# selftok-team/SelftokTokenizer

Hardware: NVIDIA H100
Metric: images/sec encode+50-step decode, 256x256/512-tok (higher is better)
Workload: dtype fp16 (IEEE-half operands on wgmma, fp32 accumulate; encoder/VQ/tables fp32)

## Files before the change

### selftoktokenizer_b200/csrc/gemm_tc.cu

```cuda
#include "common.cuh"
#include "hopper.cuh"
#include "kernels.h"

#include <stdlib.h>

namespace stk {

namespace {

using namespace hop;

constexpr int BM = 128, BN = 256, BK = 64, WK = 16;
constexpr int A_TILE_BYTES = BM * BK * 2;
constexpr int B_TILE_BYTES = BN * BK * 2;
constexpr int CONSUMERS = 2;
constexpr int NUM_THREADS = CONSUMERS * 128 + 32;
constexpr int ACC = BN / 2;

template <int NSPLIT> struct Cfg {
  static constexpr int PLANES = NSPLIT == 3 ? 2 : 1;
  static constexpr int STAGE_BYTES = PLANES * (A_TILE_BYTES + B_TILE_BYTES);
  static constexpr int STAGES = NSPLIT == 3 ? 2 : 4;
  static constexpr int SMEM_BYTES = STAGES * STAGE_BYTES + 1024  + 256 ;
};

__device__ __forceinline__ void wgmma_tile(float (&d)[ACC], uint64_t da, uint64_t db, uint32_t acc, bool fp16) {
  if (fp16) wgmma_m64n256k16_ss_f16(d, da, db, acc);
  else wgmma_m64n256k16_ss_bf16(d, da, db, acc);
}

__device__ __forceinline__ float2 ldg2(const float* p) { return *reinterpret_cast<const float2*>(p); }

template <int MODE, bool GELU>
__device__ __forceinline__ void epilogue_tile(const Epilogue& e, const float (&acc)[ACC], int64_t row0, int64_t M, int col0, int N) {
  const bool per_row_gate = MODE == EPI_RESID && e.gate && (e.gate_period > 1 || e.tab_rows);
  const bool per_row_add = MODE == EPI_STORE && e.addtab;
  const bool fp16 = e.fp16 != 0;
  int orow[2], mrow[2];
  bool rvalid[2];
#pragma unroll
  for (int r = 0; r < 2; ++r) {
    const int64_t m = row0 + 8 * r;
    rvalid[r] = m < M;
    const int mi = (int)m;
    if (e.row_map && rvalid[r]) {
      orow[r] = e.row_map[mi];
    } else if (e.plan && rvalid[r]) {
      const int b = mi / e.rpb_in;
      const int n_img = e.rpb_out - (e.plan_ctx ? e.rpb_in : e.row_off);
      orow[r] = b * e.rpb_out + plan_slot_row(mi % e.rpb_in, e.plan[2 * b], e.plan[2 * b + 1], n_img, e.plan_ctx != 0);
    } else {
      orow[r] = e.rpb_in > 0 ? (mi / e.rpb_in) * e.rpb_out + e.row_off + (mi % e.rpb_in) : mi;
    }
    if (e.tab_rows && rvalid[r]) mrow[r] = e.tab_rows[mi];
    else mrow[r] = per_row_gate ? mi % e.gate_period : (per_row_add ? mi % e.add_period : 0);
  }
#pragma unroll
  for (int j = 0; j < BN / 8; ++j) {
    const int n = col0 + 8 * j;
    if (n >= N) continue;
    const float2 bias = e.bias ? ldg2(e.bias + n) : make_float2(0.f, 0.f);
    const float2 g0 = (MODE == EPI_RESID && e.gate && !per_row_gate) ? ldg2(e.gate + n) : make_float2(1.f, 1.f);
#pragma unroll
    for (int r = 0; r < 2; ++r) {
      if (!rvalid[r]) continue;
      float2 y = make_float2(acc[4 * j + 2 * r] + bias.x, acc[4 * j + 2 * r + 1] + bias.y);
      if (GELU) y = gelu_tanh_fast2(y);
      const int64_t o = (int64_t)orow[r] * e.ldo + n;
      if (MODE == EPI_RESID) {
        const float2 res = ldg2(e.resid + o);
        const float2 gt = per_row_gate ? ldg2(e.gate + (int64_t)mrow[r] * e.gate_ld + n) : g0;
        y.x = fmaf(gt.x, y.x, res.x); y.y = fmaf(gt.y, y.y, res.y);
      }
      if (MODE == EPI_SPLIT) {
        const uint32_t hi = pack2_sat16(y.x, y.y, fp16);
        *reinterpret_cast<uint32_t*>(e.out_hi + o) = hi;
        if (e.out_lo) {
          const float lx = y.x - __bfloat162float(__float2bfloat16_rn(y.x)), ly = y.y - __bfloat162float(__float2bfloat16_rn(y.y));
          *reinterpret_cast<uint32_t*>(e.out_lo + o) = pack2_sat16(lx, ly, false);
        }
      } else {
        if (per_row_add) {
          const float2 a = ldg2(e.addtab + (int64_t)mrow[r] * e.add_ld + n);
          y.x += a.x; y.y += a.y;
        }
        *reinterpret_cast<float2*>(e.out + o) = y;
      }
    }
  }
}

__device__ __forceinline__ void epilogue_dispatch(const Epilogue& e, const float (&acc)[ACC], int64_t row0, int64_t M, int col0, int N) {
  if (e.mode == EPI_RESID) epilogue_tile<EPI_RESID, false>(e, acc, row0, M, col0, N);
  else if (e.mode == EPI_SPLIT) {
    if (e.act == ACT_GELU) epilogue_tile<EPI_SPLIT, true>(e, acc, row0, M, col0, N);
    else epilogue_tile<EPI_SPLIT, false>(e, acc, row0, M, col0, N);
  } else {
    if (e.act == ACT_GELU) epilogue_tile<EPI_STORE, true>(e, acc, row0, M, col0, N);
    else epilogue_tile<EPI_STORE, false>(e, acc, row0, M, col0, N);
  }
}

struct TcMaps {
  CUtensorMap a_hi, a_lo, b_hi, b_lo;
};

struct GemmParams {
  int64_t M;
  int N, K;
  int fp16;
  Epilogue ep;
  int conv_C = 0, conv_H = 0, conv_W = 0, conv_stride = 1;
  int raster_gm = 4;
};

__device__ __forceinline__ void tile_coords(int t, int pm_tiles, int n_tiles, int GM, int& pm, int& n_blk) {
  const int per_group = GM * n_tiles;
  const int group = t / per_group;
  const int first = group * GM;
  const int gm = min(GM, pm_tiles - first);
  const int local = t - group * per_group;
  pm = first + local % gm;
  n_blk = local / gm;
}

template <int NSPLIT, int CL, bool FP16>
__global__ void __launch_bounds__(NUM_THREADS, 1)
gemm_tc_kernel(const __grid_constant__ TcMaps maps0, const __grid_constant__ TcMaps maps1, const GemmParams p0, const GemmParams p1) {
  static_assert(NSPLIT == 1 || !FP16, "the fp16 mode is single-pass");
  using C = Cfg<NSPLIT>;
  extern __shared__ uint8_t smem_raw[];
  const uint32_t smem_base = (smem_u32(smem_raw) + 1023u) & ~1023u;
  const uint32_t bar_base = smem_base + C::STAGES * C::STAGE_BYTES;
  auto full_bar = [&](int s) { return bar_base + 8u * s; };
  auto empty_bar = [&](int s) { return bar_base + 8u * (C::STAGES + s); };

  const int warp = threadIdx.x >> 5, lane = threadIdx.x & 31;
  const uint32_t rank = CL > 1 ? cluster_ctarank() : 0;
  const int pm_tiles0 = (int)((p0.M + CL * BM - 1) / (CL * BM)), n_tiles0 = (p0.N + BN - 1) / BN;
  const int pm_tiles1 = (int)((p1.M + CL * BM - 1) / (CL * BM)), n_tiles1 = (p1.N + BN - 1) / BN;
  const int tiles0 = pm_tiles0 * n_tiles0;
  const int num_tiles = tiles0 + pm_tiles1 * n_tiles1;
  const int cluster_id = blockIdx.x / CL, num_clusters = gridDim.x / CL;

  if (warp == CONSUMERS * 4 && lane == 0) {
    tma_prefetch_desc(&maps0.a_hi);
    tma_prefetch_desc(&maps0.b_hi);
    if (NSPLIT == 3) { tma_prefetch_desc(&maps0.a_lo); tma_prefetch_desc(&maps0.b_lo); }
    if (p1.M > 0) {
      tma_prefetch_desc(&maps1.a_hi);
      tma_prefetch_desc(&maps1.b_hi);
      if (NSPLIT == 3) { tma_prefetch_desc(&maps1.a_lo); tma_prefetch_desc(&maps1.b_lo); }
    }
    for (int s = 0; s < C::STAGES; ++s) { mbar_init(full_bar(s), 1); mbar_init(empty_bar(s), CONSUMERS * CL); }
    asm volatile("fence.mbarrier_init.release.cluster;" ::: "memory");
  }
  __syncthreads();
  if (CL > 1) cluster_sync_all();

  if (warp >= CONSUMERS * 4) {
    if (warp == CONSUMERS * 4 && lane == 0) {
      int stage = 0; uint32_t phase = 0;
      const uint64_t w_policy = l2_policy_evict_last();
      for (int t = cluster_id; t < num_tiles; t += num_clusters) {
        const bool second = t >= tiles0;
        const TcMaps& mp = second ? maps1 : maps0;
        const GemmParams& pp = second ? p1 : p0;
        int pm, n_blk;
        if (second) tile_coords(t - tiles0, pm_tiles1, n_tiles1, p1.raster_gm, pm, n_blk);
        else tile_coords(t, pm_tiles0, n_tiles0, p0.raster_gm, pm, n_blk);
        const int nk = (pp.K + BK - 1) / BK;
        const int m_row = (pm * CL + (int)rank) * BM;
        const int n_row = n_blk * BN + (int)rank * (BN / CL);
        const int chunks = pp.conv_C > 0 ? pp.conv_C / BK : 1;
        int cx = 0, cy = 0, cb = 0;
        if (pp.conv_C > 0) {
          cx = m_row % pp.conv_W;
          cy = (m_row / pp.conv_W) % pp.conv_H;
          cb = m_row / (pp.conv_W * pp.conv_H);
        }
        for (int kb = 0; kb < nk; ++kb) {
          mbar_wait(empty_bar(stage), phase ^ 1);
          const uint32_t sa = smem_base + stage * C::STAGE_BYTES;
          const uint32_t sb = sa + C::PLANES * A_TILE_BYTES + (uint32_t)rank * (B_TILE_BYTES / CL);
          const uint32_t fb = full_bar(stage);
          mbar_expect_tx(fb, C::STAGE_BYTES);
          if (pp.conv_C > 0) {
            const int tap = kb / chunks, c0 = (kb - tap * chunks) * BK;
            const int dy = tap / 3, dx = tap - dy * 3;
            int x0 = cx + dx - 1, y0 = cy + dy - 1, n0 = cb;
            if (pp.conv_stride == 2) { x0 = cx + (dx >> 1); y0 = cy + (dy >> 1); n0 = cb * 4 + (dy & 1) * 2 + (dx & 1); }
            tma_load_4d(sa, &mp.a_hi, fb, c0, x0, y0, n0);
            if (NSPLIT == 3) tma_load_4d(sa + A_TILE_BYTES, &mp.a_lo, fb, c0, x0, y0, n0);
          } else {
            tma_load_2d(sa, &mp.a_hi, fb, kb * BK, m_row);
            if (NSPLIT == 3) tma_load_2d(sa + A_TILE_BYTES, &mp.a_lo, fb, kb * BK, m_row);
          }
          if (CL > 1) {
            tma_load_2d_mc(sb, &mp.b_hi, fb, kb * BK, n_row, (uint16_t)((1u << CL) - 1), w_policy);
            if (NSPLIT == 3) tma_load_2d_mc(sb + B_TILE_BYTES, &mp.b_lo, fb, kb * BK, n_row, (uint16_t)((1u << CL) - 1), w_policy);
          } else {
            tma_load_2d_hint(sb, &mp.b_hi, fb, kb * BK, n_row, w_policy);
            if (NSPLIT == 3) tma_load_2d_hint(sb + B_TILE_BYTES, &mp.b_lo, fb, kb * BK, n_row, w_policy);
          }
          if (++stage == C::STAGES) { stage = 0; phase ^= 1; }
        }
      }
    }
  } else {
    const int wg = warp >> 2;
    const bool signaller = (threadIdx.x & 127) == 0;
    auto release = [&](int s) {
      if (!signaller) return;
      if (CL == 1) mbar_arrive(empty_bar(s));
      else for (int r = 0; r < CL; ++r) mbar_arrive_cluster(empty_bar(s), (uint32_t)r);
    };
    int stage = 0; uint32_t phase = 0;
    for (int t = cluster_id; t < num_tiles; t += num_clusters) {
      const bool second = t >= tiles0;
      int pm, n_blk;
      if (second) tile_coords(t - tiles0, pm_tiles1, n_tiles1, p1.raster_gm, pm, n_blk);
      else tile_coords(t, pm_tiles0, n_tiles0, p0.raster_gm, pm, n_blk);
      const int nk = ((second ? p1.K : p0.K) + BK - 1) / BK;
      float acc[ACC];
#pragma unroll
      for (int i = 0; i < ACC; ++i) acc[i] = 0.f;
      int prev = -1;
      for (int kb = 0; kb < nk; ++kb) {
        mbar_wait(full_bar(stage), phase);
        const uint32_t sa_hi = smem_base + stage * C::STAGE_BYTES + wg * (64 * 128);
        const uint32_t sa_lo = sa_hi + A_TILE_BYTES;
        const uint32_t sb_hi = smem_base + stage * C::STAGE_BYTES + C::PLANES * A_TILE_BYTES;
        const uint32_t sb_lo = sb_hi + B_TILE_BYTES;
        wgmma_fence();
#pragma unroll
        for (int k = 0; k < BK / WK; ++k) {
          const uint32_t koff = k * WK * 2;
          const uint64_t da_hi = make_smem_desc(sa_hi + koff), db_hi = make_smem_desc(sb_hi + koff);
          wgmma_tile(acc, da_hi, db_hi, (kb > 0 || k > 0) ? 1u : 0u, FP16);
          if (NSPLIT == 3) {
            const uint64_t da_lo = make_smem_desc(sa_lo + koff), db_lo = make_smem_desc(sb_lo + koff);
            wgmma_tile(acc, da_hi, db_lo, 1u, false);
            wgmma_tile(acc, da_lo, db_hi, 1u, false);
          }
        }
        wgmma_commit();
        wgmma_wait<1>();
        if (prev >= 0) release(prev);
        prev = stage;
        if (++stage == C::STAGES) { stage = 0; phase ^= 1; }
      }
      wgmma_wait<0>();
      fence_regs(acc);
      release(prev);
      const int wl = threadIdx.x & 127;
      const int64_t row0 = (int64_t)(pm * CL + (int)rank) * BM + wg * 64 + (wl >> 5) * 16 + ((wl & 31) >> 2);
      const int col0 = n_blk * BN + 2 * (wl & 3);
      if (!second) epilogue_dispatch(p0.ep, acc, row0, p0.M, col0, p0.N);
      else epilogue_dispatch(p1.ep, acc, row0, p1.M, col0, p1.N);
    }
  }
  if (CL > 1) cluster_sync_all();
}

typedef CUresult (*EncodeTiledFn)(CUtensorMap*, CUtensorMapDataType, cuuint32_t, void*, const cuuint64_t*, const cuuint64_t*,
                                  const cuuint32_t*, const cuuint32_t*, CUtensorMapInterleave, CUtensorMapSwizzle,
                                  CUtensorMapL2promotion, CUtensorMapFloatOOBfill);
EncodeTiledFn g_encode = nullptr;
constexpr int kMaxDev = 64;
int g_num_sms_dev[kMaxDev];
bool g_attr_dev[kMaxDev];
int g_raster_gm = 4;
int g_gemm_ctas = 2;

int make_map(CUtensorMap* map, const __nv_bfloat16* ptr, int64_t rows, int K, int box_rows, int fp16) {
  cuuint64_t gdim[2] = {(cuuint64_t)K, (cuuint64_t)rows};
  cuuint64_t gstride[1] = {(cuuint64_t)K * 2};
  cuuint32_t box[2] = {(cuuint32_t)BK, (cuuint32_t)box_rows};
  cuuint32_t estr[2] = {1, 1};
  CUresult r = g_encode(map, fp16 ? CU_TENSOR_MAP_DATA_TYPE_FLOAT16 : CU_TENSOR_MAP_DATA_TYPE_BFLOAT16, 2, const_cast<__nv_bfloat16*>(ptr), gdim, gstride, box, estr,
                        CU_TENSOR_MAP_INTERLEAVE_NONE, CU_TENSOR_MAP_SWIZZLE_128B, CU_TENSOR_MAP_L2_PROMOTION_L2_256B,
                        CU_TENSOR_MAP_FLOAT_OOB_FILL_NONE);
  if (r != CUDA_SUCCESS) {
    set_error("cuTensorMapEncodeTiled failed with CUresult " + std::to_string((int)r));
    return -5;
  }
  return 0;
}

int make_map_nhwc(CUtensorMap* map, const __nv_bfloat16* ptr, int64_t B, int H, int W, int Cc, int fp16) {
  const int bw = W < BM ? W : BM;
  const int bh = (BM / bw) < H ? (BM / bw) : H;
  const int bn = BM / (bw * bh);
  cuuint64_t gdim[4] = {(cuuint64_t)Cc, (cuuint64_t)W, (cuuint64_t)H, (cuuint64_t)B};
  cuuint64_t gstride[3] = {(cuuint64_t)Cc * 2, (cuuint64_t)W * Cc * 2, (cuuint64_t)H * W * Cc * 2};
  cuuint32_t box[4] = {(cuuint32_t)BK, (cuuint32_t)bw, (cuuint32_t)bh, (cuuint32_t)bn};
  cuuint32_t estr[4] = {1, 1, 1, 1};
  CUresult r = g_encode(map, fp16 ? CU_TENSOR_MAP_DATA_TYPE_FLOAT16 : CU_TENSOR_MAP_DATA_TYPE_BFLOAT16, 4, const_cast<__nv_bfloat16*>(ptr), gdim, gstride,
                        box, estr, CU_TENSOR_MAP_INTERLEAVE_NONE, CU_TENSOR_MAP_SWIZZLE_128B, CU_TENSOR_MAP_L2_PROMOTION_L2_256B,
                        CU_TENSOR_MAP_FLOAT_OOB_FILL_NONE);
  if (r != CUDA_SUCCESS) {
    set_error("cuTensorMapEncodeTiled (NHWC) failed with CUresult " + std::to_string((int)r));
    return -5;
  }
  return 0;
}

}

int make_tensor_map_2d(CUtensorMap* map, const void* ptr, uint64_t rows, uint64_t cols, uint32_t box_rows, uint32_t box_cols,
                       int fp16) {
  STK_CHECK(g_encode, -3, "gemm_tc_init has not been called");
  cuuint64_t gdim[2] = {(cuuint64_t)cols, (cuuint64_t)rows};
  cuuint64_t gstride[1] = {(cuuint64_t)cols * 2};
  cuuint32_t box[2] = {box_cols, box_rows};
  cuuint32_t estr[2] = {1, 1};
  CUresult r = g_encode(map, fp16 ? CU_TENSOR_MAP_DATA_TYPE_FLOAT16 : CU_TENSOR_MAP_DATA_TYPE_BFLOAT16, 2, const_cast<void*>(ptr), gdim,
                        gstride, box, estr, CU_TENSOR_MAP_INTERLEAVE_NONE, CU_TENSOR_MAP_SWIZZLE_128B,
                        CU_TENSOR_MAP_L2_PROMOTION_L2_256B, CU_TENSOR_MAP_FLOAT_OOB_FILL_NONE);
  if (r != CUDA_SUCCESS) {
    set_error("cuTensorMapEncodeTiled failed with CUresult " + std::to_string((int)r));
    return -5;
  }
  return 0;
}

void gemm_tc_set_ctas(int n) { g_gemm_ctas = n == 1 ? 1 : 2; }

int gemm_tc_init() {
  int dev = 0;
  STK_CUDA(cudaGetDevice(&dev));
  STK_CHECK(dev >= 0 && dev < kMaxDev, -1, "gemm_tc: device ordinal out of range");
  if (g_encode && g_attr_dev[dev]) return 0;
  if (!g_encode) {
    void* fn = nullptr;
    cudaDriverEntryPointQueryResult qres;
    STK_CUDA(cudaGetDriverEntryPoint("cuTensorMapEncodeTiled", &fn, cudaEnableDefault, &qres));
    STK_CHECK(fn && qres == cudaDriverEntryPointSuccess, -5, "cuTensorMapEncodeTiled not available from the driver");
    const char* v = getenv("SELFTOK_GEMM_CTAS");
    if (v) g_gemm_ctas = atoi(v) == 1 ? 1 : 2;
    const char* gm = getenv("SELFTOK_GEMM_GM");
    if (gm && atoi(gm) >= 1 && atoi(gm) <= 1024) g_raster_gm = atoi(gm);
    g_encode = reinterpret_cast<EncodeTiledFn>(fn);
  }
  STK_CUDA(cudaDeviceGetAttribute(&g_num_sms_dev[dev], cudaDevAttrMultiProcessorCount, dev));
  STK_CUDA(cudaFuncSetAttribute(gemm_tc_kernel<1, 1, false>, cudaFuncAttributeMaxDynamicSharedMemorySize, Cfg<1>::SMEM_BYTES));
  STK_CUDA(cudaFuncSetAttribute(gemm_tc_kernel<1, 1, true>, cudaFuncAttributeMaxDynamicSharedMemorySize, Cfg<1>::SMEM_BYTES));
  STK_CUDA(cudaFuncSetAttribute(gemm_tc_kernel<3, 1, false>, cudaFuncAttributeMaxDynamicSharedMemorySize, Cfg<3>::SMEM_BYTES));
  STK_CUDA(cudaFuncSetAttribute(gemm_tc_kernel<1, 2, false>, cudaFuncAttributeMaxDynamicSharedMemorySize, Cfg<1>::SMEM_BYTES));
  STK_CUDA(cudaFuncSetAttribute(gemm_tc_kernel<1, 2, true>, cudaFuncAttributeMaxDynamicSharedMemorySize, Cfg<1>::SMEM_BYTES));
  STK_CUDA(cudaFuncSetAttribute(gemm_tc_kernel<3, 2, false>, cudaFuncAttributeMaxDynamicSharedMemorySize, Cfg<3>::SMEM_BYTES));
  g_attr_dev[dev] = true;
  return 0;
}

static int check_problem(const TcProblem& q, int nsplit, int fp16) {
  const Epilogue& ep = q.ep;
  STK_CHECK(q.A_hi && q.W_hi && q.M > 0 && q.N > 0 && q.K > 0, -1, "gemm_tc: bad arguments");
  STK_CHECK(nsplit == 1 || (nsplit == 3 && q.A_lo && q.W_lo), -1, "gemm_tc: nsplit must be 1, or 3 with lo planes");
  STK_CHECK(!fp16 || nsplit == 1, -1, "gemm_tc: the fp16 mode is single-pass");
  STK_CHECK(ep.act == ACT_NONE || (ep.act == ACT_GELU && ep.mode != EPI_RESID), -2,
            "gemm_tc: epilogue activation must be none, or GELU-tanh with the store / split modes");
  STK_CHECK(ep.mode != EPI_STORE || ep.addtab == nullptr || ep.add_ld % 4 == 0, -2, "gemm_tc: addtab pitch must be a multiple of 4");
  STK_CHECK(q.K % 8 == 0, -2, "gemm_tc: K must be a multiple of 8 (16-byte TMA row pitch)");
  STK_CHECK(ep.ldo % 4 == 0 && q.N % 4 == 0, -2, "gemm_tc: N and the output pitch must be multiples of 4");
  STK_CHECK(ep.mode != EPI_RESID || ep.gate == nullptr || ep.gate_ld % 4 == 0, -2, "gemm_tc: gate pitch must be a multiple of 4");
  if (q.conv_C > 0) {
    STK_CHECK(q.conv_C % BK == 0 && q.K == 9 * q.conv_C, -2, "gemm_tc conv: channels must be a multiple of 64 and K = 9 C");
    STK_CHECK(q.conv_W > 0 && q.conv_H > 0 && (q.conv_W % BM == 0 || BM % q.conv_W == 0), -2, "gemm_tc conv: image width must divide or be a multiple of 128");
    const int64_t hw = (int64_t)q.conv_H * q.conv_W;
    STK_CHECK(q.M % hw == 0 && (hw % BM == 0 || BM % hw == 0) && (q.conv_W >= BM || hw < BM || q.conv_H % (BM / q.conv_W) == 0), -2,
              "gemm_tc conv: 128-pixel tiles must be part of a row, whole rows of one image, or whole images");
    STK_CHECK(q.conv_stride == 1 || (q.conv_stride == 2 && hw % BM == 0), -2, "gemm_tc conv: stride 2 needs >= 128 output pixels per image");
  }
  return 0;
}

static int make_maps(TcMaps* m, const TcProblem& q, int nsplit, int fp16, int b_box) {
  const bool conv = q.conv_C > 0;
  const int64_t imgs = conv ? q.M / ((int64_t)q.conv_H * q.conv_W) * (q.conv_stride == 2 ? 4 : 1) : 0;
  if (conv) STK_TRY(make_map_nhwc(&m->a_hi, q.A_hi, imgs, q.conv_H, q.conv_W, q.conv_C, fp16));
  else STK_TRY(make_map(&m->a_hi, q.A_hi, q.M, q.K, BM, fp16));
  STK_TRY(make_map(&m->b_hi, q.W_hi, q.N, q.K, b_box, fp16));
  if (nsplit == 3) {
    if (conv) STK_TRY(make_map_nhwc(&m->a_lo, q.A_lo, imgs, q.conv_H, q.conv_W, q.conv_C, fp16));
    else STK_TRY(make_map(&m->a_lo, q.A_lo, q.M, q.K, BM, fp16));
    STK_TRY(make_map(&m->b_lo, q.W_lo, q.N, q.K, b_box, fp16));
  } else {
    m->a_lo = m->a_hi; m->b_lo = m->b_hi;
  }
  return 0;
}

template <int NSPLIT, int CL, bool FP16>
static int launch_kernel(const TcMaps& m0, const TcMaps& m1, const GemmParams& p0, const GemmParams& p1, int clusters, cudaStream_t s) {
  cudaLaunchConfig_t cfg = {};
  cfg.gridDim = dim3(CL * clusters);
  cfg.blockDim = dim3(NUM_THREADS);
  cfg.dynamicSmemBytes = Cfg<NSPLIT>::SMEM_BYTES;
  cfg.stream = s;
  cudaLaunchAttribute attr[1];
  attr[0].id = cudaLaunchAttributeClusterDimension;
  attr[0].val.clusterDim.x = CL; attr[0].val.clusterDim.y = 1; attr[0].val.clusterDim.z = 1;
  cfg.attrs = attr;
  cfg.numAttrs = 1;
  STK_CUDA(cudaLaunchKernelEx(&cfg, gemm_tc_kernel<NSPLIT, CL, FP16>, m0, m1, p0, p1));
  count_launch();
  return 0;
}

template <int CL>
static int launch_cl(const TcMaps& m0, const TcMaps& m1, const GemmParams& p0, const GemmParams& p1, int clusters, int nsplit, int fp16,
                     cudaStream_t s) {
  if (nsplit == 3) return launch_kernel<3, CL, false>(m0, m1, p0, p1, clusters, s);
  if (fp16) return launch_kernel<1, CL, true>(m0, m1, p0, p1, clusters, s);
  return launch_kernel<1, CL, false>(m0, m1, p0, p1, clusters, s);
}

int launch_gemm_tc_grouped(const TcProblem* probs, int n, int nsplit, cudaStream_t s, int fp16) {
  STK_TRY(gemm_tc_init());
  STK_CHECK(probs && (n == 1 || n == 2), -1, "gemm_tc: one or two problems per launch");
  int dev = 0;
  STK_CUDA(cudaGetDevice(&dev));
  const int g_num_sms = g_num_sms_dev[dev];
  for (int i = 0; i < n; ++i) STK_TRY(check_problem(probs[i], nsplit, fp16));
  const int CL = g_gemm_ctas == 2 && g_num_sms >= 2 ? 2 : 1;
  TcMaps m0, m1;
  STK_TRY(make_maps(&m0, probs[0], nsplit, fp16, BN / CL));
  auto mk_params = [&](const TcProblem& q) {
    GemmParams g{q.M, q.N, q.K, fp16, q.ep};
    g.conv_C = q.conv_C; g.conv_H = q.conv_H; g.conv_W = q.conv_W; g.conv_stride = q.conv_stride;
    g.raster_gm = g_raster_gm;
    return g;
  };
  GemmParams p0 = mk_params(probs[0]);
  GemmParams p1 = p0;
  p1.M = 0;
  m1 = m0;
  int tiles = (int)((probs[0].M + CL * BM - 1) / (CL * BM)) * ((probs[0].N + BN - 1) / BN);
  if (n == 2) {
    STK_TRY(make_maps(&m1, probs[1], nsplit, fp16, BN / CL));
    p1 = mk_params(probs[1]);
    tiles += (int)((probs[1].M + CL * BM - 1) / (CL * BM)) * ((probs[1].N + BN - 1) / BN);
  }
  const int clusters = tiles < g_num_sms / CL ? tiles : g_num_sms / CL;
  if (CL == 2) return launch_cl<2>(m0, m1, p0, p1, clusters, nsplit, fp16, s);
  return launch_cl<1>(m0, m1, p0, p1, clusters, nsplit, fp16, s);
}

int launch_gemm_tc(const __nv_bfloat16* A_hi, const __nv_bfloat16* A_lo, const __nv_bfloat16* W_hi,
                   const __nv_bfloat16* W_lo, int64_t M, int N, int K, int nsplit, const Epilogue& ep,
                   cudaStream_t s, int fp16) {
  TcProblem q{A_hi, A_lo, W_hi, W_lo, M, N, K, ep};
  return launch_gemm_tc_grouped(&q, 1, nsplit, s, fp16);
}

}
```

### selftoktokenizer_b200/csrc/hopper.cuh

```cuda
#pragma once
#include <cuda.h>
#include <stdint.h>

namespace stk {
namespace hop {

__device__ __forceinline__ uint32_t smem_u32(const void* p) { return (uint32_t)__cvta_generic_to_shared(p); }

__device__ __forceinline__ void mbar_init(uint32_t bar, uint32_t count) {
  asm volatile("mbarrier.init.shared::cta.b64 [%0], %1;" ::"r"(bar), "r"(count) : "memory");
}
__device__ __forceinline__ void mbar_expect_tx(uint32_t bar, uint32_t bytes) {
  asm volatile("mbarrier.arrive.expect_tx.shared::cta.b64 _, [%0], %1;" ::"r"(bar), "r"(bytes) : "memory");
}
__device__ __forceinline__ void mbar_arrive(uint32_t bar) {
  asm volatile("mbarrier.arrive.shared::cta.b64 _, [%0];" ::"r"(bar) : "memory");
}
__device__ __forceinline__ void mbar_arrive_cluster(uint32_t local_bar, uint32_t rank) {
  asm volatile(
      "{\n\t.reg .b32 ra;\n\t"
      "mapa.shared::cluster.u32 ra, %0, %1;\n\t"
      "mbarrier.arrive.shared::cluster.b64 _, [ra];\n\t}"
      ::"r"(local_bar), "r"(rank) : "memory");
}
constexpr uint32_t kSuspendHintNs = 20000;
__device__ __forceinline__ bool mbar_try_wait(uint32_t bar, uint32_t parity) {
  uint32_t ok;
  asm volatile(
      "{\n\t.reg .pred p;\n\t"
      "mbarrier.try_wait.parity.shared::cta.b64 p, [%1], %2, %3;\n\t"
      "selp.u32 %0, 1, 0, p;\n\t}"
      : "=r"(ok) : "r"(bar), "r"(parity), "r"(kSuspendHintNs) : "memory");
  return ok != 0;
}
__device__ __forceinline__ void mbar_wait(uint32_t bar, uint32_t parity) {
  if (mbar_try_wait(bar, parity)) return;
  const long long t0 = clock64();
  uint32_t spins = 0;
  while (!mbar_try_wait(bar, parity)) {
    if ((++spins & 0x3ff) == 0 && clock64() - t0 > 8000000000LL) __trap();
  }
}

__device__ __forceinline__ void tma_prefetch_desc(const CUtensorMap* map) {
  asm volatile("prefetch.tensormap [%0];" ::"l"(reinterpret_cast<uint64_t>(map)) : "memory");
}
__device__ __forceinline__ void tma_load_2d(uint32_t dst, const CUtensorMap* map, uint32_t bar, int c0, int c1) {
  asm volatile(
      "cp.async.bulk.tensor.2d.shared::cluster.global.mbarrier::complete_tx::bytes [%0], [%1, {%3, %4}], [%2];"
      ::"r"(dst), "l"(reinterpret_cast<uint64_t>(map)), "r"(bar), "r"(c0), "r"(c1) : "memory");
}
__device__ __forceinline__ void tma_load_4d(uint32_t dst, const CUtensorMap* map, uint32_t bar, int c0, int c1, int c2, int c3) {
  asm volatile(
      "cp.async.bulk.tensor.4d.shared::cluster.global.mbarrier::complete_tx::bytes [%0], [%1, {%3, %4, %5, %6}], [%2];"
      ::"r"(dst), "l"(reinterpret_cast<uint64_t>(map)), "r"(bar), "r"(c0), "r"(c1), "r"(c2), "r"(c3) : "memory");
}
__device__ __forceinline__ void tma_load_2d_mc(uint32_t dst, const CUtensorMap* map, uint32_t bar, int c0, int c1, uint16_t mask,
                                               uint64_t policy) {
  asm volatile(
      "cp.async.bulk.tensor.2d.shared::cluster.global.mbarrier::complete_tx::bytes.multicast::cluster.L2::cache_hint"
      " [%0], [%1, {%3, %4}], [%2], %5, %6;"
      ::"r"(dst), "l"(reinterpret_cast<uint64_t>(map)), "r"(bar), "r"(c0), "r"(c1), "h"(mask), "l"(policy) : "memory");
}
__device__ __forceinline__ void tma_load_2d_hint(uint32_t dst, const CUtensorMap* map, uint32_t bar, int c0, int c1, uint64_t policy) {
  asm volatile(
      "cp.async.bulk.tensor.2d.shared::cluster.global.mbarrier::complete_tx::bytes.L2::cache_hint [%0], [%1, {%3, %4}], [%2], %5;"
      ::"r"(dst), "l"(reinterpret_cast<uint64_t>(map)), "r"(bar), "r"(c0), "r"(c1), "l"(policy) : "memory");
}
__device__ __forceinline__ uint64_t l2_policy_evict_last() {
  uint64_t pol;
  asm volatile("createpolicy.fractional.L2::evict_last.b64 %0, 1.0;" : "=l"(pol));
  return pol;
}

__device__ __forceinline__ uint32_t cluster_ctarank() {
  uint32_t r;
  asm volatile("mov.u32 %0, %%cluster_ctarank;" : "=r"(r));
  return r;
}
__device__ __forceinline__ void cluster_sync_all() {
  asm volatile("barrier.cluster.arrive.release.aligned;\n\tbarrier.cluster.wait.acquire.aligned;" ::: "memory");
}

__device__ __forceinline__ uint64_t make_smem_desc(uint32_t smem_addr) {
  uint64_t d = 0;
  d |= (uint64_t)((smem_addr >> 4) & 0x3FFF);
  d |= (uint64_t)1 << 16;
  d |= (uint64_t)(1024 >> 4) << 32;
  d |= (uint64_t)1 << 62;
  return d;
}
__device__ __forceinline__ void wgmma_fence() { asm volatile("wgmma.fence.sync.aligned;" ::: "memory"); }
__device__ __forceinline__ void wgmma_commit() { asm volatile("wgmma.commit_group.sync.aligned;" ::: "memory"); }
template <int N>
__device__ __forceinline__ void wgmma_wait() { asm volatile("wgmma.wait_group.sync.aligned %0;" ::"n"(N) : "memory"); }
template <int R>
__device__ __forceinline__ void fence_regs(float (&d)[R]) {
#pragma unroll
  for (int i = 0; i < R; ++i) asm volatile("" : "+f"(d[i])::"memory");
}

#define STK_WGMMA_SS_N256(NAME, T)                                                                                   \
  __device__ __forceinline__ void NAME(float (&d)[128], uint64_t da, uint64_t db, uint32_t accumulate) { \
    asm volatile("{\n\t.reg .pred p;\n\tsetp.ne.b32 p, %130, 0;\n\t"                                             \
                 "wgmma.mma_async.sync.aligned.m64n256k16.f32." T "." T " "                                             \
                 "{%0, %1, %2, %3, %4, %5, %6, %7, %8, %9, %10, %11, %12, %13, %14, %15, %16, %17, %18, %19, %20, %21, %22, %23, %24, %25, %26, %27, %28, %29, %30, %31, %32, %33, %34, %35, %36, %37, %38, %39, %40, %41, %42, %43, %44, %45, %46, %47, %48, %49, %50, %51, %52, %53, %54, %55, %56, %57, %58, %59, %60, %61, %62, %63, %64, %65, %66, %67, %68, %69, %70, %71, %72, %73, %74, %75, %76, %77, %78, %79, %80, %81, %82, %83, %84, %85, %86, %87, %88, %89, %90, %91, %92, %93, %94, %95, %96, %97, %98, %99, %100, %101, %102, %103, %104, %105, %106, %107, %108, %109, %110, %111, %112, %113, %114, %115, %116, %117, %118, %119, %120, %121, %122, %123, %124, %125, %126, %127}, "  \
                 "%128, %129, p, 1, 1, 0, 0;\n\t}"                                                                  \
                 : "+f"(d[0]), "+f"(d[1]), "+f"(d[2]), "+f"(d[3]), "+f"(d[4]), "+f"(d[5]), "+f"(d[6]), "+f"(d[7]), "+f"(d[8]), "+f"(d[9]), "+f"(d[10]), "+f"(d[11]), "+f"(d[12]), "+f"(d[13]), "+f"(d[14]), "+f"(d[15]), "+f"(d[16]), "+f"(d[17]), "+f"(d[18]), "+f"(d[19]), "+f"(d[20]), "+f"(d[21]), "+f"(d[22]), "+f"(d[23]), "+f"(d[24]), "+f"(d[25]), "+f"(d[26]), "+f"(d[27]), "+f"(d[28]), "+f"(d[29]), "+f"(d[30]), "+f"(d[31]), "+f"(d[32]), "+f"(d[33]), "+f"(d[34]), "+f"(d[35]), "+f"(d[36]), "+f"(d[37]), "+f"(d[38]), "+f"(d[39]), "+f"(d[40]), "+f"(d[41]), "+f"(d[42]), "+f"(d[43]), "+f"(d[44]), "+f"(d[45]), "+f"(d[46]), "+f"(d[47]), "+f"(d[48]), "+f"(d[49]), "+f"(d[50]), "+f"(d[51]), "+f"(d[52]), "+f"(d[53]), "+f"(d[54]), "+f"(d[55]), "+f"(d[56]), "+f"(d[57]), "+f"(d[58]), "+f"(d[59]), "+f"(d[60]), "+f"(d[61]), "+f"(d[62]), "+f"(d[63]), "+f"(d[64]), "+f"(d[65]), "+f"(d[66]), "+f"(d[67]), "+f"(d[68]), "+f"(d[69]), "+f"(d[70]), "+f"(d[71]), "+f"(d[72]), "+f"(d[73]), "+f"(d[74]), "+f"(d[75]), "+f"(d[76]), "+f"(d[77]), "+f"(d[78]), "+f"(d[79]), "+f"(d[80]), "+f"(d[81]), "+f"(d[82]), "+f"(d[83]), "+f"(d[84]), "+f"(d[85]), "+f"(d[86]), "+f"(d[87]), "+f"(d[88]), "+f"(d[89]), "+f"(d[90]), "+f"(d[91]), "+f"(d[92]), "+f"(d[93]), "+f"(d[94]), "+f"(d[95]), "+f"(d[96]), "+f"(d[97]), "+f"(d[98]), "+f"(d[99]), "+f"(d[100]), "+f"(d[101]), "+f"(d[102]), "+f"(d[103]), "+f"(d[104]), "+f"(d[105]), "+f"(d[106]), "+f"(d[107]), "+f"(d[108]), "+f"(d[109]), "+f"(d[110]), "+f"(d[111]), "+f"(d[112]), "+f"(d[113]), "+f"(d[114]), "+f"(d[115]), "+f"(d[116]), "+f"(d[117]), "+f"(d[118]), "+f"(d[119]), "+f"(d[120]), "+f"(d[121]), "+f"(d[122]), "+f"(d[123]), "+f"(d[124]), "+f"(d[125]), "+f"(d[126]), "+f"(d[127]) \
                 : "l"(da), "l"(db), "r"(accumulate));                                                                         \
  }
STK_WGMMA_SS_N256(wgmma_m64n256k16_ss_bf16, "bf16")
STK_WGMMA_SS_N256(wgmma_m64n256k16_ss_f16, "f16")

#define STK_WGMMA_SS_N64(NAME, T)                                                                                   \
  __device__ __forceinline__ void NAME(float (&d)[32], uint64_t da, uint64_t db, uint32_t accumulate) { \
    asm volatile("{\n\t.reg .pred p;\n\tsetp.ne.b32 p, %34, 0;\n\t"                                             \
                 "wgmma.mma_async.sync.aligned.m64n64k16.f32." T "." T " "                                             \
                 "{%0, %1, %2, %3, %4, %5, %6, %7, %8, %9, %10, %11, %12, %13, %14, %15, %16, %17, %18, %19, %20, %21, %22, %23, %24, %25, %26, %27, %28, %29, %30, %31}, "  \
                 "%32, %33, p, 1, 1, 0, 0;\n\t}"                                                                  \
                 : "+f"(d[0]), "+f"(d[1]), "+f"(d[2]), "+f"(d[3]), "+f"(d[4]), "+f"(d[5]), "+f"(d[6]), "+f"(d[7]), "+f"(d[8]), "+f"(d[9]), "+f"(d[10]), "+f"(d[11]), "+f"(d[12]), "+f"(d[13]), "+f"(d[14]), "+f"(d[15]), "+f"(d[16]), "+f"(d[17]), "+f"(d[18]), "+f"(d[19]), "+f"(d[20]), "+f"(d[21]), "+f"(d[22]), "+f"(d[23]), "+f"(d[24]), "+f"(d[25]), "+f"(d[26]), "+f"(d[27]), "+f"(d[28]), "+f"(d[29]), "+f"(d[30]), "+f"(d[31]) \
                 : "l"(da), "l"(db), "r"(accumulate));                                                                         \
  }
STK_WGMMA_SS_N64(wgmma_m64n64k16_ss_bf16, "bf16")
STK_WGMMA_SS_N64(wgmma_m64n64k16_ss_f16, "f16")

#define STK_WGMMA_RS_N64(NAME, T)                                                                                   \
  __device__ __forceinline__ void NAME(float (&d)[32], const uint32_t (&a)[4], uint64_t db, uint32_t accumulate) { \
    asm volatile("{\n\t.reg .pred p;\n\tsetp.ne.b32 p, %37, 0;\n\t"                                             \
                 "wgmma.mma_async.sync.aligned.m64n64k16.f32." T "." T " "                                             \
                 "{%0, %1, %2, %3, %4, %5, %6, %7, %8, %9, %10, %11, %12, %13, %14, %15, %16, %17, %18, %19, %20, %21, %22, %23, %24, %25, %26, %27, %28, %29, %30, %31}, "  \
                 "{%32, %33, %34, %35}, %36, p, 1, 1, 1;\n\t}"                                                                  \
                 : "+f"(d[0]), "+f"(d[1]), "+f"(d[2]), "+f"(d[3]), "+f"(d[4]), "+f"(d[5]), "+f"(d[6]), "+f"(d[7]), "+f"(d[8]), "+f"(d[9]), "+f"(d[10]), "+f"(d[11]), "+f"(d[12]), "+f"(d[13]), "+f"(d[14]), "+f"(d[15]), "+f"(d[16]), "+f"(d[17]), "+f"(d[18]), "+f"(d[19]), "+f"(d[20]), "+f"(d[21]), "+f"(d[22]), "+f"(d[23]), "+f"(d[24]), "+f"(d[25]), "+f"(d[26]), "+f"(d[27]), "+f"(d[28]), "+f"(d[29]), "+f"(d[30]), "+f"(d[31]) \
                 : "r"(a[0]), "r"(a[1]), "r"(a[2]), "r"(a[3]), "l"(db), "r"(accumulate));                                                                         \
  }
STK_WGMMA_RS_N64(wgmma_m64n64k16_rs_bf16, "bf16")
STK_WGMMA_RS_N64(wgmma_m64n64k16_rs_f16, "f16")

}
}
```

Before: 8.689.

## Rebalance warp-specialized registers and prefetch epilogue residuals into L2 during mainloop

Grows the producer from one warp to a full warpgroup so setmaxnreg can shrink producer registers and grow consumer registers for the 128-float accumulators. Epilogue row mapping is computed before the mainloop, and residual rows are L2-prefetched a few k-blocks before the tile finishes. The epilogue now batches its bias, residual and gate loads into chunks before the math so the memory latency overlaps. It adds a profiling script. The risks are register pressure from the batched loads, and the extra producer warps lowering occupancy if the kernel runs 2 CTAs per SM.

```diff
diff --git a/profiles/gemm_stages.py b/profiles/gemm_stages.py
--- /dev/null
+++ b/profiles/gemm_stages.py
@@ -0,0 +1,100 @@
+import json
+import os
+import subprocess
+import sys
+import tempfile
+
+import torch
+from torch.profiler import ProfilerActivity, profile
+
+REPO = os.path.dirname(os.path.dirname(os.path.abspath(__file__)))
+sys.path.insert(0, REPO)
+from selftoktokenizer_b200 import capi, config as C, schedule as S, synth
+
+B, STEPS = 64, 50
+STAGES = ["x_embedder", "qkv", "proj", "fc1", "fc2", "final_layer"]
+
+
+def gpu_info():
+    q = "name,power.limit,clocks.sm,clocks.max.sm"
+    r = subprocess.run(["nvidia-smi", f"--query-gpu={q}", "--format=csv,noheader"], capture_output=True, text=True, check=True)
+    name, plim, sm, smax = [v.strip() for v in r.stdout.strip().splitlines()[0].split(",")]
+    return {"name": name, "power_limit": plim, "sm_clock": sm, "sm_clock_max": smax}
+
+
+def stage_flops(d):
+    tb = S.make_tables(d.K, d.stages, d.k_per_stage, STEPS)
+    D, N, L = d.dit_hidden, d.n_img, d.dit_depth
+    Kp = d.in_channels * d.dit_patch * d.dit_patch
+    f = dict.fromkeys(STAGES, 0.0)
+    for i in range(STEPS):
+        kc = int(tb.k[i]) + 1
+        f["x_embedder"] += 2.0 * B * N * Kp * D
+        f["final_layer"] += 2.0 * B * N * D * Kp
+        for j in range(L):
+            rows_ctx = 0 if j == L - 1 else kc
+            f["qkv"] += 2.0 * B * (N + kc) * D * 3 * D
+            f["proj"] += 2.0 * B * (N + rows_ctx) * D * D
+            f["fc1"] += 2.0 * B * (N + rows_ctx) * D * 4 * D
+            f["fc2"] += 2.0 * B * (N + rows_ctx) * 4 * D * D
+    return f
+
+
+def gemm_kernel_times(trace_path):
+    ev = json.load(open(trace_path))["traceEvents"]
+    k = [e for e in ev if e.get("cat") == "kernel" and "gemm_tc_kernel" in e.get("name", "")]
+    k.sort(key=lambda e: e["ts"])
+    return [e["dur"] / 1000.0 for e in k]
+
+
+def run(prec, tmp):
+    d = C.FULL
+    dev = torch.device("cuda:0")
+    eng = capi.Engine(d, synth.synth_state_dict(d, device=dev), device=dev, precision=prec, steps=STEPS)
+    g = torch.Generator().manual_seed(0)
+    tok = torch.randint(0, d.codebook_size, (B, d.K), generator=g).to(dev)
+    noise = torch.randn(B, d.in_channels, d.latent, d.latent, generator=g).to(dev)
+    eng.set_use_graph(False)
+    eng.decode(tok, noise)
+    torch.cuda.synchronize()
+    with profile(activities=[ProfilerActivity.CUDA]) as prof:
+        eng.decode(tok, noise)
+        torch.cuda.synchronize()
+    path = os.path.join(tmp, f"gemm_stages_{prec}.pt.trace.json")
+    prof.export_chrome_trace(path)
+    eng.close()
+    times = gemm_kernel_times(path)
+    per_step = 2 + 4 * d.dit_depth
+    assert len(times) == STEPS * per_step, f"{len(times)} gemm_tc_kernel launches, expected {STEPS} x {per_step}"
+    ms = dict.fromkeys(STAGES, 0.0)
+    for i, t in enumerate(times):
+        p = i % per_step
+        ms["x_embedder" if p == 0 else "final_layer" if p == per_step - 1 else STAGES[1 + (p - 1) % 4]] += t
+    flops = stage_flops(d)
+    total = sum(ms.values())
+    rows = {s: {"ms": ms[s], "tflop": flops[s] / 1e12, "tflops": flops[s] / (ms[s] / 1e3) / 1e12, "share": ms[s] / total}
+            for s in STAGES}
+    rows["all"] = {"ms": total, "tflop": sum(flops.values()) / 1e12,
+                   "tflops": sum(flops.values()) / (total / 1e3) / 1e12, "share": 1.0}
+    return rows
+
+
+def main():
+    if not torch.cuda.is_available():
+        raise SystemExit("gemm_stages.py needs a CUDA device")
+    precs = sys.argv[1:] or ["fp16", "bf16x3"]
+    out = {"gpu": gpu_info(), "batch": B, "steps": STEPS}
+    with tempfile.TemporaryDirectory() as tmp:
+        for prec in precs:
+            rows = run(prec, tmp)
+            out[prec] = rows
+            print(f"\n{prec}: gemm_tc_kernel per stage, B = {B}, {STEPS}-step decode, graphs off")
+            print(f"{'stage':<12}{'ms':>10}{'TFLOP':>10}{'TFLOP/s':>10}{'share':>8}")
+            for s, r in rows.items():
+                print(f"{s:<12}{r['ms']:>10.1f}{r['tflop']:>10.1f}{r['tflops']:>10.1f}{r['share']:>8.3f}")
+    out["gpu_after"] = gpu_info()
+    print(json.dumps(out))
+
+
+if __name__ == "__main__":
+    main()
diff --git a/selftoktokenizer_b200/csrc/gemm_tc.cu b/selftoktokenizer_b200/csrc/gemm_tc.cu
--- a/selftoktokenizer_b200/csrc/gemm_tc.cu
+++ b/selftoktokenizer_b200/csrc/gemm_tc.cu
@@ -14,8 +14,10 @@
 constexpr int A_TILE_BYTES = BM * BK * 2;
 constexpr int B_TILE_BYTES = BN * BK * 2;
 constexpr int CONSUMERS = 2;
-constexpr int NUM_THREADS = CONSUMERS * 128 + 32;
+constexpr int NUM_THREADS = CONSUMERS * 128 + 128;
+constexpr int PRODUCER_REGS = 40, CONSUMER_REGS = 232;
 constexpr int ACC = BN / 2;
+constexpr int kPrefetchKBlocks = 4;
 
 template <int NSPLIT> struct Cfg {
   static constexpr int PLANES = NSPLIT == 3 ? 2 : 1;
@@ -31,73 +33,114 @@
 
 __device__ __forceinline__ float2 ldg2(const float* p) { return *reinterpret_cast<const float2*>(p); }
 
+struct EpiRows {
+  int orow[2], mrow[2];
+  bool valid[2];
+};
+
+__device__ __forceinline__ EpiRows epilogue_rows(const Epilogue& e, int64_t row0, int64_t M) {
+  const bool per_row_gate = e.mode == EPI_RESID && e.gate && (e.gate_period > 1 || e.tab_rows);
+  const bool per_row_add = e.mode == EPI_STORE && e.addtab;
+  EpiRows rw;
+#pragma unroll
+  for (int r = 0; r < 2; ++r) {
+    const int64_t m = row0 + 8 * r;
+    rw.valid[r] = m < M;
+    const int mi = (int)m;
+    rw.orow[r] = 0;
+    if (e.row_map && rw.valid[r]) {
+      rw.orow[r] = e.row_map[mi];
+    } else if (e.plan && rw.valid[r]) {
+      const int b = mi / e.rpb_in;
+      const int n_img = e.rpb_out - (e.plan_ctx ? e.rpb_in : e.row_off);
+      rw.orow[r] = b * e.rpb_out + plan_slot_row(mi % e.rpb_in, e.plan[2 * b], e.plan[2 * b + 1], n_img, e.plan_ctx != 0);
+    } else if (rw.valid[r]) {
+      rw.orow[r] = e.rpb_in > 0 ? (mi / e.rpb_in) * e.rpb_out + e.row_off + (mi % e.rpb_in) : mi;
+    }
+    if (e.tab_rows && rw.valid[r]) rw.mrow[r] = e.tab_rows[mi];
+    else rw.mrow[r] = per_row_gate ? mi % e.gate_period : (per_row_add ? mi % e.add_period : 0);
+  }
+  return rw;
+}
+
+__device__ __forceinline__ void epilogue_prefetch(const Epilogue& e, const EpiRows& rw, int col0, int N) {
+  if (e.mode != EPI_RESID) return;
+  const int c0 = col0 & ~(BN - 1);
+  const int q = (col0 >> 1) & 3;
+#pragma unroll
+  for (int r = 0; r < 2; ++r) {
+#pragma unroll
+    for (int h = 0; h < 2; ++h) {
+      const int n = c0 + 32 * (2 * q + h);
+      if (rw.valid[r] && n < N) prefetch_l2(e.resid + (int64_t)rw.orow[r] * e.ldo + n);
+    }
+  }
+}
+
 template <int MODE, bool GELU>
-__device__ __forceinline__ void epilogue_tile(const Epilogue& e, const float (&acc)[ACC], int64_t row0, int64_t M, int col0, int N) {
+__device__ __forceinline__ void epilogue_tile(const Epilogue& e, const float (&acc)[ACC], const EpiRows& rw, int col0, int N) {
+  constexpr int CH = MODE == EPI_RESID ? 4 : 8;
   const bool per_row_gate = MODE == EPI_RESID && e.gate && (e.gate_period > 1 || e.tab_rows);
   const bool per_row_add = MODE == EPI_STORE && e.addtab;
   const bool fp16 = e.fp16 != 0;
-  int orow[2], mrow[2];
-  bool rvalid[2];
-#pragma unroll
-  for (int r = 0; r < 2; ++r) {
-    const int64_t m = row0 + 8 * r;
-    rvalid[r] = m < M;
-    const int mi = (int)m;
-    if (e.row_map && rvalid[r]) {
-      orow[r] = e.row_map[mi];
-    } else if (e.plan && rvalid[r]) {
-      const int b = mi / e.rpb_in;
-      const int n_img = e.rpb_out - (e.plan_ctx ? e.rpb_in : e.row_off);
-      orow[r] = b * e.rpb_out + plan_slot_row(mi % e.rpb_in, e.plan[2 * b], e.plan[2 * b + 1], n_img, e.plan_ctx != 0);
-    } else {
-      orow[r] = e.rpb_in > 0 ? (mi / e.rpb_in) * e.rpb_out + e.row_off + (mi % e.rpb_in) : mi;
-    }
-    if (e.tab_rows && rvalid[r]) mrow[r] = e.tab_rows[mi];
-    else mrow[r] = per_row_gate ? mi % e.gate_period : (per_row_add ? mi % e.add_period : 0);
-  }
-#pragma unroll
-  for (int j = 0; j < BN / 8; ++j) {
-    const int n = col0 + 8 * j;
-    if (n >= N) continue;
-    const float2 bias = e.bias ? ldg2(e.bias + n) : make_float2(0.f, 0.f);
-    const float2 g0 = (MODE == EPI_RESID && e.gate && !per_row_gate) ? ldg2(e.gate + n) : make_float2(1.f, 1.f);
-#pragma unroll
-    for (int r = 0; r < 2; ++r) {
-      if (!rvalid[r]) continue;
-      float2 y = make_float2(acc[4 * j + 2 * r] + bias.x, acc[4 * j + 2 * r + 1] + bias.y);
-      if (GELU) y = gelu_tanh_fast2(y);
-      const int64_t o = (int64_t)orow[r] * e.ldo + n;
-      if (MODE == EPI_RESID) {
-        const float2 res = ldg2(e.resid + o);
-        const float2 gt = per_row_gate ? ldg2(e.gate + (int64_t)mrow[r] * e.gate_ld + n) : g0;
-        y.x = fmaf(gt.x, y.x, res.x); y.y = fmaf(gt.y, y.y, res.y);
+  const float2 zero = make_float2(0.f, 0.f), one = make_float2(1.f, 1.f);
+#pragma unroll
+  for (int c = 0; c < BN / 8; c += CH) {
+    float2 bias[CH], res[2][CH], gt[2][CH], add[2][CH];
+#pragma unroll
+    for (int i = 0; i < CH; ++i) {
+      const int n = col0 + 8 * (c + i);
+      const bool in = n < N;
+      bias[i] = e.bias && in ? ldg2(e.bias + n) : zero;
+#pragma unroll
+      for (int r = 0; r < 2; ++r) {
+        const bool v = in && rw.valid[r];
+        const int64_t o = (int64_t)rw.orow[r] * e.ldo + n;
+        if (MODE == EPI_RESID) {
+          res[r][i] = v ? ldg2(e.resid + o) : zero;
+          gt[r][i] = v && e.gate ? ldg2(per_row_gate ? e.gate + (int64_t)rw.mrow[r] * e.gate_ld + n : e.gate + n) : one;
+        }
+        if (MODE == EPI_STORE) add[r][i] = v && per_row_add ? ldg2(e.addtab + (int64_t)rw.mrow[r] * e.add_ld + n) : zero;
       }
-      if (MODE == EPI_SPLIT) {
-        const uint32_t hi = pack2_sat16(y.x, y.y, fp16);
-        *reinterpret_cast<uint32_t*>(e.out_hi + o) = hi;
-        if (e.out_lo) {
-          const float lx = y.x - __bfloat162float(__float2bfloat16_rn(y.x)), ly = y.y - __bfloat162float(__float2bfloat16_rn(y.y));
-          *reinterpret_cast<uint32_t*>(e.out_lo + o) = pack2_sat16(lx, ly, false);
-        }
-      } else {
-        if (per_row_add) {
-          const float2 a = ldg2(e.addtab + (int64_t)mrow[r] * e.add_ld + n);
-          y.x += a.x; y.y += a.y;
-        }
-        *reinterpret_cast<float2*>(e.out + o) = y;
+    }
+#pragma unroll
+    for (int i = 0; i < CH; ++i) {
+      const int j = c + i;
+      const int n = col0 + 8 * j;
+      if (n >= N) continue;
+#pragma unroll
+      for (int r = 0; r < 2; ++r) {
+        if (!rw.valid[r]) continue;
+        float2 y = make_float2(acc[4 * j + 2 * r] + bias[i].x, acc[4 * j + 2 * r + 1] + bias[i].y);
+        if (GELU) y = gelu_tanh_fast2(y);
+        const int64_t o = (int64_t)rw.orow[r] * e.ldo + n;
+        if (MODE == EPI_RESID) {
+          y.x = fmaf(gt[r][i].x, y.x, res[r][i].x); y.y = fmaf(gt[r][i].y, y.y, res[r][i].y);
+        }
+        if (MODE == EPI_SPLIT) {
+          const uint32_t hi = pack2_sat16(y.x, y.y, fp16);
+          *reinterpret_cast<uint32_t*>(e.out_hi + o) = hi;
+          if (e.out_lo) {
+            const float lx = y.x - __bfloat162float(__float2bfloat16_rn(y.x)), ly = y.y - __bfloat162float(__float2bfloat16_rn(y.y));
+            *reinterpret_cast<uint32_t*>(e.out_lo + o) = pack2_sat16(lx, ly, false);
+          }
+        } else {
+          if (per_row_add) { y.x += add[r][i].x; y.y += add[r][i].y; }
+          *reinterpret_cast<float2*>(e.out + o) = y;
+        }
       }
     }
   }
 }
 
-__device__ __forceinline__ void epilogue_dispatch(const Epilogue& e, const float (&acc)[ACC], int64_t row0, int64_t M, int col0, int N) {
-  if (e.mode == EPI_RESID) epilogue_tile<EPI_RESID, false>(e, acc, row0, M, col0, N);
+__device__ __forceinline__ void epilogue_dispatch(const Epilogue& e, const float (&acc)[ACC], const EpiRows& rw, int col0, int N) {
+  if (e.mode == EPI_RESID) epilogue_tile<EPI_RESID, false>(e, acc, rw, col0, N);
   else if (e.mode == EPI_SPLIT) {
-    if (e.act == ACT_GELU) epilogue_tile<EPI_SPLIT, true>(e, acc, row0, M, col0, N);
-    else epilogue_tile<EPI_SPLIT, false>(e, acc, row0, M, col0, N);
+    if (e.act == ACT_GELU) epilogue_tile<EPI_SPLIT, true>(e, acc, rw, col0, N);
+    else epilogue_tile<EPI_SPLIT, false>(e, acc, rw, col0, N);
   } else {
-    if (e.act == ACT_GELU) epilogue_tile<EPI_STORE, true>(e, acc, row0, M, col0, N);
-    else epilogue_tile<EPI_STORE, false>(e, acc, row0, M, col0, N);
+    if (e.act == ACT_GELU) epilogue_tile<EPI_STORE, true>(e, acc, rw, col0, N);
+    else epilogue_tile<EPI_STORE, false>(e, acc, rw, col0, N);
   }
 }
 
@@ -159,6 +202,7 @@
   if (CL > 1) cluster_sync_all();
 
   if (warp >= CONSUMERS * 4) {
+    setmaxnreg_dec<PRODUCER_REGS>();
     if (warp == CONSUMERS * 4 && lane == 0) {
       int stage = 0; uint32_t phase = 0;
       const uint64_t w_policy = l2_policy_evict_last();
@@ -208,6 +252,7 @@
       }
     }
   } else {
+    setmaxnreg_inc<CONSUMER_REGS>();
     const int wg = warp >> 2;
     const bool signaller = (threadIdx.x & 127) == 0;
     auto release = [&](int s) {
@@ -222,6 +267,11 @@
       if (second) tile_coords(t - tiles0, pm_tiles1, n_tiles1, p1.raster_gm, pm, n_blk);
       else tile_coords(t, pm_tiles0, n_tiles0, p0.raster_gm, pm, n_blk);
       const int nk = ((second ? p1.K : p0.K) + BK - 1) / BK;
+      const int wl = threadIdx.x & 127;
+      const int64_t row0 = (int64_t)(pm * CL + (int)rank) * BM + wg * 64 + (wl >> 5) * 16 + ((wl & 31) >> 2);
+      const int col0 = n_blk * BN + 2 * (wl & 3);
+      const EpiRows rw = second ? epilogue_rows(p1.ep, row0, p1.M) : epilogue_rows(p0.ep, row0, p0.M);
+      const int pf_kb = nk > kPrefetchKBlocks ? nk - kPrefetchKBlocks : 0;
       float acc[ACC];
 #pragma unroll
       for (int i = 0; i < ACC; ++i) acc[i] = 0.f;
@@ -245,6 +295,10 @@
           }
         }
         wgmma_commit();
+        if (kb == pf_kb) {
+          if (!second) epilogue_prefetch(p0.ep, rw, col0, p0.N);
+          else epilogue_prefetch(p1.ep, rw, col0, p1.N);
+        }
         wgmma_wait<1>();
         if (prev >= 0) release(prev);
         prev = stage;
@@ -253,11 +307,8 @@
       wgmma_wait<0>();
       fence_regs(acc);
       release(prev);
-      const int wl = threadIdx.x & 127;
-      const int64_t row0 = (int64_t)(pm * CL + (int)rank) * BM + wg * 64 + (wl >> 5) * 16 + ((wl & 31) >> 2);
-      const int col0 = n_blk * BN + 2 * (wl & 3);
-      if (!second) epilogue_dispatch(p0.ep, acc, row0, p0.M, col0, p0.N);
-      else epilogue_dispatch(p1.ep, acc, row0, p1.M, col0, p1.N);
+      if (!second) epilogue_dispatch(p0.ep, acc, rw, col0, p0.N);
+      else epilogue_dispatch(p1.ep, acc, rw, col0, p1.N);
     }
   }
   if (CL > 1) cluster_sync_all();
diff --git a/selftoktokenizer_b200/csrc/hopper.cuh b/selftoktokenizer_b200/csrc/hopper.cuh
--- a/selftoktokenizer_b200/csrc/hopper.cuh
+++ b/selftoktokenizer_b200/csrc/hopper.cuh
@@ -73,6 +73,13 @@
   return pol;
 }
 
+template <int R> __device__ __forceinline__ void setmaxnreg_inc() { asm volatile("setmaxnreg.inc.sync.aligned.u32 %0;" ::"n"(R)); }
+template <int R> __device__ __forceinline__ void setmaxnreg_dec() { asm volatile("setmaxnreg.dec.sync.aligned.u32 %0;" ::"n"(R)); }
+
+__device__ __forceinline__ void prefetch_l2(const void* p) {
+  asm volatile("prefetch.global.L2 [%0];" ::"l"(reinterpret_cast<uint64_t>(p)));
+}
+
 __device__ __forceinline__ uint32_t cluster_ctarank() {
   uint32_t r;
   asm volatile("mov.u32 %0, %%cluster_ctarank;" : "=r"(r));
```

Result: faster. 9.936, median of 6 (+14.3%).
